# ToniChopp/ECAMP

Hardware: AMD Instinct MI355X
Metric: pretrain image-report pairs/sec (ViT-B/16, 224^2, seq=128) (higher is better)
Workload: dtype bf16

## Files before the change

### ecamp_amd/csrc/attention.h

```cpp
#pragma once
#include "common.h"

struct AttnArgs {
    const void* q; const void* k; const void* v; void* o;
    const void* dout; void* dq; void* dk; void* dv;
    float* lse; float* delta;
    const int32_t* key_mask;
    long q_sb, q_st, q_sh, k_sb, k_st, k_sh, v_sb, v_st, v_sh, o_sb, o_st, o_sh;
    long dq_sb, dq_st, dq_sh, dk_sb, dk_st, dk_sh, dv_sb, dv_st, dv_sh, do_sb, do_st, do_sh;
    int B, H, Tq, Tk;
    float scale, drop_p;
    uint64_t seed, offset;
    unsigned char* drop_bits;
};

#define NEG_BIG (-1.0e30f)

#define LDS_MAX (160 * 1024)

static inline int attn_kch(int Tk) { return Tk <= 64 ? 1 : Tk <= 128 ? 2 : Tk <= 256 ? 4 : 0; }

static inline size_t head_lds_bytes(int Tq, int Tk, int hd, bool backward, bool bits) {
    const int nkp = ((Tk + 15) / 16 + 1) / 2, nqp = ((Tq + 15) / 16 + 1) / 2;
    const size_t prow = (size_t)(backward && nqp > nkp ? nqp : nkp) * 32;
    return 2 * prow * (2 * hd) + (backward ? 3 : 1) * prow * sizeof(float) + (backward && bits ? 32 * prow : 0);
}

enum AttnFamily { ATTN_HEAD, ATTN_RESIDENT_FWD, ATTN_STREAM, ATTN_LONG, ATTN_F32 };
typedef void (*AttnKernel)(AttnArgs);
struct AttnLaunch {
    AttnFamily family;
    int n, block;
    struct Kernel { AttnKernel fn; dim3 grid; size_t lds, optin; } k[2];
};
#define ATTN_HD_SWITCH(hd, F, ...) ((hd) == 32 ? F<32>(__VA_ARGS__) : (hd) == 64 ? F<64>(__VA_ARGS__) : F<128>(__VA_ARGS__))

ECAMP_HIDDEN AttnLaunch attn16_select(int B, int H, int Tq, int Tk, int hd, bool mask_or_dropout, bool bits, bool backward);
ECAMP_HIDDEN void attn_launch(const AttnLaunch& l, const AttnArgs& a, hipStream_t st);
void attn_set_head_mode(int on);
```

### ecamp_amd/csrc/attention_bf16.hip

```cpp
#include "attention.h"
#include <type_traits>

#ifdef ATTN_TS
__device__ long long attn_ts_buf[8 * 8192];
#define ATTN_STAMP(i) do { if (threadIdx.x == 0 && blockIdx.x < 8192) attn_ts_buf[blockIdx.x * 8 + (i)] = wall_clock64(); } while (0)
#else
#define ATTN_STAMP(i) do { } while (0)
#endif

typedef __attribute__((ext_vector_type(4))) short v4s16;
typedef hw_h16x8 bf16x8_t;

#define MFMA(a, b, c) ECAMP_MFMA_16x16x32(a, b, c)

#define ATTN_LOG2E 1.4426950408889634f
#define ATTN_LN2 0.6931471805599453f
__device__ __forceinline__ float attn_exp2(float x) { return __builtin_amdgcn_exp2f(x); }

template <int HD> struct TileCfg { static constexpr int PB = HD * 2 + 32; static constexpr int BYTES = 64 * PB; };

template <int HD>
__device__ __forceinline__ void stage_tile(unsigned char* lds, const bf16_t* base, long st, int r0, int nrows, int tid) {
    constexpr int CPR = HD / 8, PB = TileCfg<HD>::PB;
#pragma unroll
// ... 269 lines not shown
            const int4 km = *reinterpret_cast<const int4*>(KM + jt * 16 + 4 * g);
            const int kmv[4] = {km.x, km.y, km.z, km.w};
            float ds[4], dm[4] = {1.f, 1.f, 1.f, 1.f};
            if (a.drop_p > 0.f) attn_drop4(a, (uint64_t)bh * a.Tq + qi, c * 64 + jt * 16 + 4 * g, inv_keep, dm);
#pragma unroll
            for (int r = 0; r < 4; ++r) {
                const bool ok = qok && kmv[r] != 0;
                float p = ok ? attn_exp2(fmaf(s[r], sc2, -lse2)) : 0.f;
                ds[r] = p * (dp[r] * dm[r] - dl);
            }
            ptile_write4(st, li, jt * 16 + 4 * g, ds);
        }
        __builtin_amdgcn_s_waitcnt(0xc07f);
        __builtin_amdgcn_wave_barrier();
#pragma unroll
        for (int kk = 0; kk < 2; ++kk) {
            bf16x8 sf = ptile_frag(st, li, kk * 4 + g);
#pragma unroll
            for (int dt = 0; dt < HD / 16; ++dt) dq[dt] = MFMA(frag_tr<HD>(KT, dt * 16, kk * 32, lane), sf, dq[dt]);
        }
    }
    if (qok) {
#pragma unroll
        for (int dt = 0; dt < HD / 16; ++dt) store4(dqb + (long)qi * a.dq_st + dt * 16 + 4 * g, dq[dt], a.scale);
    }
}

template <int HD, int KCH>
__global__ __launch_bounds__(256) void attn16_bwd_dq_kernel(AttnArgs a) {
    const int nact = min(4, (a.Tq - (int)blockIdx.x * 64 + 15) >> 4);
    if (nact < 4) {
        if ((int)(threadIdx.x >> 6) >= nact) return;
        attn16_bwd_dq_body<HD, KCH, true>(a, nact * 64);
    } else {
        attn16_bwd_dq_body<HD, KCH, false>(a, 256);
    }
}

template <int HD, bool PART>
__device__ __forceinline__ void attn16_bwd_dkv_body(const AttnArgs& a, int nthr) {
    extern __shared__ __attribute__((aligned(16))) unsigned char smem[];
    unsigned char* QT = smem;
    unsigned char* GT = smem + TileCfg<HD>::BYTES;
    unsigned char* PT = smem + 2 * TileCfg<HD>::BYTES;
    unsigned char* ST = PT + 4 * 2048;
    float* LS = reinterpret_cast<float*>(ST + 4 * 2048);
    const int tid = threadIdx.x, lane = tid & 63, wave = tid >> 6, li = lane & 15, g = lane >> 4;
    const int b = blockIdx.y / a.H, h = blockIdx.y % a.H;
    const int j0 = blockIdx.x * 64 + wave * 16;
    const long bh = (long)b * a.H + h;
    const bf16_t* qb = reinterpret_cast<const bf16_t*>(a.q) + b * a.q_sb + h * a.q_sh;
    const bf16_t* kb = reinterpret_cast<const bf16_t*>(a.k) + b * a.k_sb + h * a.k_sh;
    const bf16_t* vb = reinterpret_cast<const bf16_t*>(a.v) + b * a.v_sb + h * a.v_sh;
    const bf16_t* gb = reinterpret_cast<const bf16_t*>(a.dout) + b * a.do_sb + h * a.do_sh;
    bf16_t* dkb = reinterpret_cast<bf16_t*>(a.dk) + b * a.dk_sb + h * a.dk_sh;
    bf16_t* dvb = reinterpret_cast<bf16_t*>(a.dv) + b * a.dv_sb + h * a.dv_sh;

    bf16x8 kf[HD / 32], vf[HD / 32];
    load_row_frags<HD>(kf, kb, a.k_st, j0, a.Tk, lane);
    load_row_frags<HD>(vf, vb, a.v_st, j0, a.Tk, lane);
    const int kj = j0 + li;
    const bool jok = kj < a.Tk && (a.key_mask == nullptr || a.key_mask[(long)b * a.Tk + kj] != 0);
    const float inv_keep = a.drop_p > 0.f ? 1.0f / (1.0f - a.drop_p) : 1.0f, sc2 = a.scale * ATTN_LOG2E;
    f32x4 dk[HD / 16], dv[HD / 16];
#pragma unroll
    for (int dt = 0; dt < HD / 16; ++dt) dk[dt] = dv[dt] = (f32x4){0.f, 0.f, 0.f, 0.f};
    unsigned char* pt = PT + wave * 2048;
    unsigned char* st = ST + wave * 2048;
    const int nqc = (a.Tq + 63) / 64;
#pragma unroll 1
    for (int c = 0; c < nqc; ++c) {
        __syncthreads();
        if (PART) {
            stage_tile_n<HD>(QT, qb, a.q_st, c * 64, a.Tq, tid, nthr);
            stage_tile_n<HD>(GT, gb, a.do_st, c * 64, a.Tq, tid, nthr);
        } else {
            stage_tile<HD>(QT, qb, a.q_st, c * 64, a.Tq, tid);
            stage_tile<HD>(GT, gb, a.do_st, c * 64, a.Tq, tid);
        }
        if (tid < 64) {
            const int i = c * 64 + tid;
            LS[tid] = i < a.Tq ? a.lse[bh * a.Tq + i] * ATTN_LOG2E : 0.f;
            LS[64 + tid] = i < a.Tq ? a.delta[bh * a.Tq + i] : 0.f;
        }
        __syncthreads();
#pragma unroll
        for (int it = 0; it < 4; ++it) {
            f32x4 s = {0.f, 0.f, 0.f, 0.f}, dp = {0.f, 0.f, 0.f, 0.f};
#pragma unroll
            for (int ks = 0; ks < HD / 32; ++ks) {
                s = MFMA(frag_rows<HD>(QT, it * 16 + li, ks * 4 + g), kf[ks], s);
                dp = MFMA(frag_rows<HD>(GT, it * 16 + li, ks * 4 + g), vf[ks], dp);
            }
            float pd[4], ds[4], dm[4] = {1.f, 1.f, 1.f, 1.f};
            if (a.drop_p > 0.f) attn_drop4_col(a, (uint64_t)bh * a.Tq + (c * 64 + it * 16 + 4 * g), kj, li, inv_keep, dm);
            const f32x4 lse4 = *reinterpret_cast<const f32x4*>(LS + it * 16 + 4 * g);
            const f32x4 dl4 = *reinterpret_cast<const f32x4*>(LS + 64 + it * 16 + 4 * g);
#pragma unroll
            for (int r = 0; r < 4; ++r) {
                int i = c * 64 + it * 16 + 4 * g + r;
                bool ok = jok && i < a.Tq;
                float p = ok ? attn_exp2(fmaf(s[r], sc2, -lse4[r])) : 0.f;
                pd[r] = p * dm[r];
                ds[r] = p * (dp[r] * dm[r] - dl4[r]);
            }
            ptile_write4(pt, li, it * 16 + 4 * g, pd);
            ptile_write4(st, li, it * 16 + 4 * g, ds);
        }
        __builtin_amdgcn_s_waitcnt(0xc07f);
        __builtin_amdgcn_wave_barrier();
#pragma unroll
        for (int kk = 0; kk < 2; ++kk) {
            bf16x8 pf = ptile_frag(pt, li, kk * 4 + g), sf = ptile_frag(st, li, kk * 4 + g);
#pragma unroll
            for (int dt = 0; dt < HD / 16; ++dt) {
                dv[dt] = MFMA(frag_tr<HD>(GT, dt * 16, kk * 32, lane), pf, dv[dt]);
                dk[dt] = MFMA(frag_tr<HD>(QT, dt * 16, kk * 32, lane), sf, dk[dt]);
            }
        }
    }
    if (kj < a.Tk) {
#pragma unroll
        for (int dt = 0; dt < HD / 16; ++dt) {
            store4(dkb + (long)kj * a.dk_st + dt * 16 + 4 * g, dk[dt], a.scale);
            store4(dvb + (long)kj * a.dv_st + dt * 16 + 4 * g, dv[dt], 1.0f);
        }
    }
}

template <int HD>
__global__ __launch_bounds__(256) void attn16_bwd_dkv_kernel(AttnArgs a) {
    const int nact = min(4, (a.Tk - (int)blockIdx.x * 64 + 15) >> 4);
    if (nact < 4) {
        if ((int)(threadIdx.x >> 6) >= nact) return;
        attn16_bwd_dkv_body<HD, true>(a, nact * 64);
    } else {
        attn16_bwd_dkv_body<HD, false>(a, 256);
    }
}

template <int HD, int KCH>
__global__ __launch_bounds__(256) void attn16r_fwd_kernel(AttnArgs a) {
    extern __shared__ __attribute__((aligned(16))) unsigned char smem[];
    constexpr int TB = TileCfg<HD>::BYTES;
    unsigned char* KT = smem;
    unsigned char* VT = smem + KCH * TB;
    unsigned char* PT = smem + 2 * KCH * TB;
    const int tid = threadIdx.x, lane = tid & 63, wave = tid >> 6, li = lane & 15, g = lane >> 4;
    const int b = blockIdx.x / a.H, h = blockIdx.x % a.H;
    const long bh = blockIdx.x;
    const bf16_t* qb = reinterpret_cast<const bf16_t*>(a.q) + b * a.q_sb + h * a.q_sh;
    const bf16_t* kb = reinterpret_cast<const bf16_t*>(a.k) + b * a.k_sb + h * a.k_sh;
    const bf16_t* vb = reinterpret_cast<const bf16_t*>(a.v) + b * a.v_sb + h * a.v_sh;
    bf16_t* ob = reinterpret_cast<bf16_t*>(a.o) + b * a.o_sb + h * a.o_sh;
#pragma unroll
    for (int c = 0; c < KCH; ++c) {
        stage_tile<HD>(KT + c * TB, kb, a.k_st, c * 64, a.Tk, tid);
        stage_tile<HD>(VT + c * TB, vb, a.v_st, c * 64, a.Tk, tid);
    }
    __syncthreads();
    const float inv_keep = a.drop_p > 0.f ? 1.0f / (1.0f - a.drop_p) : 1.0f;
    unsigned char* pt = PT + wave * 2048;
    unsigned long long kok = 0ull;
#pragma unroll
    for (int t = 0; t < KCH * 4; ++t)
#pragma unroll
        for (int r = 0; r < 4; ++r) {
            int j = t * 16 + 4 * g + r;
            bool ok = j < a.Tk && (a.key_mask == nullptr || a.key_mask[(long)b * a.Tk + j] != 0);
            kok |= (unsigned long long)(ok ? 1 : 0) << (t * 4 + r);
        }
    for (int q0 = wave * 16; q0 < a.Tq; q0 += 64) {
        bf16x8 qf[HD / 32];
        load_row_frags<HD>(qf, qb, a.q_st, q0, a.Tq, lane);
        f32x4 s[KCH * 4];
#pragma unroll
        for (int c = 0; c < KCH; ++c)
#pragma unroll
            for (int jt = 0; jt < 4; ++jt) {
                f32x4 acc = {0.f, 0.f, 0.f, 0.f};
#pragma unroll
                for (int ks = 0; ks < HD / 32; ++ks) acc = MFMA(frag_rows<HD>(KT + c * TB, jt * 16 + li, ks * 4 + g), qf[ks], acc);
                s[c * 4 + jt] = acc;
            }
        float mx = NEG_BIG;
#pragma unroll
        for (int t = 0; t < KCH * 4; ++t)
#pragma unroll
            for (int r = 0; r < 4; ++r) {
                s[t][r] = ((kok >> (t * 4 + r)) & 1ull) ? s[t][r] * (a.scale * ATTN_LOG2E) : NEG_BIG;
                mx = fmaxf(mx, s[t][r]);
            }
        mx = red4_max(mx);
        const float mxs = fmaxf(mx, -1e29f);
        float sum = 0.f;
#pragma unroll
        for (int t = 0; t < KCH * 4; ++t)
#pragma unroll
            for (int r = 0; r < 4; ++r) {
                float p = attn_exp2(s[t][r] - mxs);
                s[t][r] = p;
                sum += p;
            }
        sum = red4_sum(sum);
        const int qi = q0 + li;
        if (g == 0 && qi < a.Tq) a.lse[bh * a.Tq + qi] = (mx + __log2f(sum)) * ATTN_LN2;
        const float inv = 1.0f / sum;
        f32x4 o[HD / 16];
#pragma unroll
        for (int dt = 0; dt < HD / 16; ++dt) o[dt] = (f32x4){0.f, 0.f, 0.f, 0.f};
#pragma unroll
        for (int c = 0; c < KCH; ++c) {
#pragma unroll
            for (int jt = 0; jt < 4; ++jt) {
                float p[4];
#pragma unroll
                for (int r = 0; r < 4; ++r) p[r] = s[c * 4 + jt][r] * inv;
                if (a.drop_p > 0.f) {
                    float dm[4];
                    attn_drop4(a, (uint64_t)bh * a.Tq + qi, c * 64 + jt * 16 + 4 * g, inv_keep, dm);
#pragma unroll
                    for (int r = 0; r < 4; ++r) p[r] *= dm[r];
                }
                ptile_write4(pt, li, jt * 16 + 4 * g, p);
            }
            __builtin_amdgcn_s_waitcnt(0xc07f);
            __builtin_amdgcn_wave_barrier();
#pragma unroll
            for (int kk = 0; kk < 2; ++kk) {
                bf16x8 pf = ptile_frag(pt, li, kk * 4 + g);
#pragma unroll
                for (int dt = 0; dt < HD / 16; ++dt) o[dt] = MFMA(frag_tr<HD>(VT + c * TB, dt * 16, kk * 32, lane), pf, o[dt]);
            }
            __builtin_amdgcn_s_waitcnt(0xc07f);
            __builtin_amdgcn_wave_barrier();
        }
        if (qi < a.Tq) {
#pragma unroll
            for (int dt = 0; dt < HD / 16; ++dt) store4(ob + (long)qi * a.o_st + dt * 16 + 4 * g, o[dt], 1.0f);
        }
    }
}

template <int HD> struct HeadCfg {
    static constexpr int RB = HD * 2, CPR = HD / 8;
    static constexpr unsigned long long KEYS = HD == 32 ? 0x3033030132330101ull : HD == 64 ? 0x6056142366024421ull : 0xE0CA8436CE0A3864ull;
};
template <int HD> __device__ __forceinline__ int hswz(int row) { return (int)((HeadCfg<HD>::KEYS >> (4 * (row & 15))) & 15ull); }
template <int HD> __device__ __forceinline__ unsigned haddr(int row, int chunk) {
    return (unsigned)(row * HeadCfg<HD>::RB + ((chunk ^ hswz<HD>(row)) << 4));
}
template <int HD>
__device__ __forceinline__ void head_stage(unsigned char* img, const bf16_t* base, long st, int nrows, int prow, int tid, int nthr) {
    constexpr int CPR = HeadCfg<HD>::CPR;
    const int n = prow * CPR;
    for (int i0 = tid; i0 < n; i0 += 4 * nthr) {
        uint4 v[4];
#pragma unroll
        for (int u = 0; u < 4; ++u) {
            const int idx = i0 + u * nthr, row = idx / CPR, ch = idx % CPR;
            v[u] = (idx < n && row < nrows) ? *reinterpret_cast<const uint4*>(base + (long)row * st + ch * 8) : make_uint4(0, 0, 0, 0);
        }
#pragma unroll
        for (int u = 0; u < 4; ++u) {
            const int idx = i0 + u * nthr, row = idx / CPR, ch = idx % CPR;
            if (idx < n) *reinterpret_cast<uint4*>(img + haddr<HD>(row, ch)) = v[u];
        }
    }
}
template <int HD, int U>
__device__ __forceinline__ void head_stage_pair(unsigned char* imgA, const bf16_t* baseA, long stA, unsigned char* imgB, const bf16_t* baseB, long stB,
                                                int nrows, int prow, int tid, int nthr) {
    constexpr int CPR = HeadCfg<HD>::CPR;
    const int n = prow * CPR;
    for (int i0 = tid; i0 < n; i0 += U * nthr) {
        uint4 va[U], vb[U];
#pragma unroll
        for (int u = 0; u < U; ++u) {
            const int idx = i0 + u * nthr, row = idx / CPR, ch = idx % CPR;
            const bool in = idx < n && row < nrows;
            va[u] = in ? *reinterpret_cast<const uint4*>(baseA + (long)row * stA + ch * 8) : make_uint4(0, 0, 0, 0);
            vb[u] = in ? *reinterpret_cast<const uint4*>(baseB + (long)row * stB + ch * 8) : make_uint4(0, 0, 0, 0);
        }
#pragma unroll
        for (int u = 0; u < U; ++u) {
            const int idx = i0 + u * nthr, row = idx / CPR, ch = idx % CPR;
            if (idx < n) {
                *reinterpret_cast<uint4*>(imgA + haddr<HD>(row, ch)) = va[u];
                *reinterpret_cast<uint4*>(imgB + haddr<HD>(row, ch)) = vb[u];
            }
        }
    }
}
typedef float f32x2 __attribute__((ext_vector_type(2)));
__device__ __forceinline__ f32x2 hexp2(f32x2 x) { return (f32x2){attn_exp2(x[0]), attn_exp2(x[1])}; }
__device__ __forceinline__ uint32_t hpk(f32x2 v) { return pack_bf16x2(v[0], v[1]); }
__device__ __forceinline__ bf16x8 hpack8(const float (&v)[8]) {
    const uint4 u = make_uint4(pack_bf16x2(v[0], v[1]), pack_bf16x2(v[2], v[3]), pack_bf16x2(v[4], v[5]), pack_bf16x2(v[6], v[7]));
    return __builtin_bit_cast(bf16x8, u);
}
__device__ __forceinline__ void head_key_bias(float* KB, const AttnArgs& a, int b, int prow, int tid, int nthr) {
    for (int j = tid; j < prow; j += nthr)
        KB[j] = (j < a.Tk && (a.key_mask == nullptr || a.key_mask[(long)b * a.Tk + j] != 0)) ? 0.f : NEG_BIG;
}
template <int HD> struct HeadOff {
    unsigned fr[HD / 32];
    unsigned tr[HD / 16];
    __device__ __forceinline__ HeadOff(int li, int g) {
#pragma unroll
        for (int ks = 0; ks < HD / 32; ++ks) fr[ks] = haddr<HD>(li, ks * 4 + g);
#pragma unroll
        for (int dt = 0; dt < HD / 16; ++dt) {
            const int cb = (dt * 16 + (li & 3) * 4) * 2;
            tr[dt] = haddr<HD>(4 * g + (li >> 2), cb >> 4) + (cb & 15);
        }
    }
};
template <int HD> __device__ __forceinline__ bf16x8 hfr(const unsigned char* img, const HeadOff<HD>& o, int t, int ks) {
    return *reinterpret_cast<const bf16x8*>(img + o.fr[ks] + t * (16 * HeadCfg<HD>::RB));
}
template <int HD> __device__ __forceinline__ bf16x8 htr(const unsigned char* img, const HeadOff<HD>& o, int pp, int dt) {
    const unsigned char* p = img + o.tr[dt] + pp * (32 * HeadCfg<HD>::RB);
    v4s16 lo = __builtin_amdgcn_ds_read_tr16_b64_v4i16((v4s16 __attribute__((address_space(3)))*)(p));
    v4s16 hi = __builtin_amdgcn_ds_read_tr16_b64_v4i16((v4s16 __attribute__((address_space(3)))*)(p + 16 * HeadCfg<HD>::RB));
    return (bf16x8){lo[0], lo[1], lo[2], lo[3], hi[0], hi[1], hi[2], hi[3]};
}

template <int HD, int FLAGS>
__global__ __launch_bounds__(512, 4) void attn_head_fwd_kernel(AttnArgs a) {
    extern __shared__ __attribute__((aligned(16))) unsigned char smem[];
    constexpr int RB = HeadCfg<HD>::RB;
    const int nthr = blockDim.x, nw = nthr >> 6;
    const int nkp = (((a.Tk + 15) >> 4) + 1) >> 1, prow = nkp * 32;
    const int pfull = FLAGS ? 0 : a.Tk >> 5;
    unsigned char* KI = smem;
    unsigned char* VI = smem + prow * RB;
    float* KB = reinterpret_cast<float*>(smem + 2 * prow * RB);
    const int tid = threadIdx.x, lane = tid & 63, wave = tid >> 6, li = lane & 15, g = lane >> 4;
    const int b = blockIdx.x / a.H, h = blockIdx.x % a.H;
    const long bh = blockIdx.x;
    const bf16_t* qb = reinterpret_cast<const bf16_t*>(a.q) + b * a.q_sb + h * a.q_sh;
    const bf16_t* kb = reinterpret_cast<const bf16_t*>(a.k) + b * a.k_sb + h * a.k_sh;
    const bf16_t* vb = reinterpret_cast<const bf16_t*>(a.v) + b * a.v_sb + h * a.v_sh;
    bf16_t* ob = reinterpret_cast<bf16_t*>(a.o) + b * a.o_sb + h * a.o_sh;
    bf16x8 qf[HD / 32];
    if (wave * 16 < a.Tq) load_row_frags<HD>(qf, qb, a.q_st, wave * 16, a.Tq, lane);
    head_stage_pair<HD, 4>(KI, kb, a.k_st, VI, vb, a.v_st, a.Tk, prow, tid, nthr);
    head_key_bias(KB, a, b, prow, tid, nthr);
    __syncthreads();
    const HeadOff<HD> off(li, g);
    const float sc2 = a.scale * ATTN_LOG2E;
    const float inv_keep = a.drop_p > 0.f ? 1.0f / (1.0f - a.drop_p) : 1.0f;
    for (int q0 = wave * 16; q0 < a.Tq; q0 += nw * 16) {
        auto scores = [&](int t, bool biased) {
            f32x4 acc = {0.f, 0.f, 0.f, 0.f};
#pragma unroll
            for (int ks = 0; ks < HD / 32; ++ks) acc = MFMA(hfr<HD>(KI, off, t, ks), qf[ks], acc);
            if (biased) {
                const f32x4 kb4 = *reinterpret_cast<const f32x4*>(KB + t * 16 + 4 * g);
#pragma unroll
                for (int r = 0; r < 4; ++r) acc[r] = fmaf(acc[r], sc2, kb4[r]);
            } else {
#pragma unroll
                for (int r = 0; r < 4; ++r) acc[r] *= sc2;
            }
            return acc;
        };
        float mx = NEG_BIG;
#pragma unroll 2
        for (int pp = 0; pp < pfull; ++pp) {
            const f32x4 s0 = scores(2 * pp, false), s1 = scores(2 * pp + 1, false);
            mx = fmaxf(fmaxf(fmaxf(mx, fmaxf(s0[0], s0[1])), fmaxf(s0[2], s0[3])), fmaxf(fmaxf(s1[0], s1[1]), fmaxf(s1[2], s1[3])));
        }
#pragma unroll 1
        for (int pp = pfull; pp < nkp; ++pp) {
            const f32x4 s0 = scores(2 * pp, true), s1 = scores(2 * pp + 1, true);
            mx = fmaxf(fmaxf(fmaxf(mx, fmaxf(s0[0], s0[1])), fmaxf(s0[2], s0[3])), fmaxf(fmaxf(s1[0], s1[1]), fmaxf(s1[2], s1[3])));
        }
        mx = red4_max(mx);
        const float mxs = fmaxf(mx, -1e29f);
        const int qi = q0 + li;
        float sum = 0.f;
        f32x4 o[HD / 16];
#pragma unroll
        for (int dt = 0; dt < HD / 16; ++dt) o[dt] = (f32x4){0.f, 0.f, 0.f, 0.f};
        auto pair = [&](int pp, bool biased) {
            const f32x4 s0 = scores(2 * pp, biased), s1 = scores(2 * pp + 1, biased);
            float p[8];
#pragma unroll
            for (int r = 0; r < 4; ++r) {
                p[r] = attn_exp2(s0[r] - mxs);
                p[4 + r] = attn_exp2(s1[r] - mxs);
                sum += p[r] + p[4 + r];
            }
            if (FLAGS && a.drop_p > 0.f) {
                float dm[4], dn[4];
                if ((a.Tk & 7) == 0) {
                    const bool odd = (g & 1) != 0;
                    const uint64_t e8 = ((((uint64_t)bh * a.Tq + qi) * (uint64_t)a.Tk) >> 3) + (uint64_t)(pp * 4 + (odd ? 2 : 0) + (g >> 1));
                    const uint4 P = philox4x32(a.seed, a.offset, e8);
                    const uint32_t r0 = (uint32_t)__builtin_amdgcn_ds_swizzle((int)(odd ? P.x : P.z), 0x401f);
                    const uint32_t r1 = (uint32_t)__builtin_amdgcn_ds_swizzle((int)(odd ? P.y : P.w), 0x401f);
                    const uint32_t wa0 = odd ? r0 : P.x, wa1 = odd ? r1 : P.y, wb0 = odd ? P.z : r0, wb1 = odd ? P.w : r1;
                    const uint32_t thr = dropout_thr(a.drop_p);
                    dm[0] = dropout_pick(wa0, 0, thr, inv_keep); dm[1] = dropout_pick(wa0, 1, thr, inv_keep);
                    dm[2] = dropout_pick(wa1, 0, thr, inv_keep); dm[3] = dropout_pick(wa1, 1, thr, inv_keep);
                    dn[0] = dropout_pick(wb0, 0, thr, inv_keep); dn[1] = dropout_pick(wb0, 1, thr, inv_keep);
                    dn[2] = dropout_pick(wb1, 0, thr, inv_keep); dn[3] = dropout_pick(wb1, 1, thr, inv_keep);
                } else {
                    attn_drop4(a, (uint64_t)bh * a.Tq + qi, pp * 32 + 4 * g, inv_keep, dm);
                    attn_drop4(a, (uint64_t)bh * a.Tq + qi, pp * 32 + 16 + 4 * g, inv_keep, dn);
                }
                unsigned bits = 0;
#pragma unroll
                for (int r = 0; r < 4; ++r) {
                    p[r] *= dm[r];
                    p[4 + r] *= dn[r];
                    bits |= (dm[r] != 0.f ? 1u << r : 0u) | (dn[r] != 0.f ? 16u << r : 0u);
                }
                if (a.drop_bits && qi < a.Tq) a.drop_bits[(((long)bh * a.Tq + qi) * 4 + g) * 8 + pp] = (unsigned char)bits;
            }
            const bf16x8 pf = hpack8(p);
#pragma unroll
            for (int dt = 0; dt < HD / 16; ++dt) o[dt] = MFMA(htr<HD>(VI, off, pp, dt), pf, o[dt]);
        };
#pragma unroll 2
        for (int pp = 0; pp < pfull; ++pp) pair(pp, false);
#pragma unroll 1
        for (int pp = pfull; pp < nkp; ++pp) pair(pp, true);
        sum = red4_sum(sum);
        if (qi < a.Tq) {
            if (g == 0) a.lse[bh * a.Tq + qi] = (mxs + __log2f(sum)) * ATTN_LN2;
            const float inv = sum > 0.f ? 1.0f / sum : 0.f;
#pragma unroll
            for (int dt = 0; dt < HD / 16; ++dt) store4(ob + (long)qi * a.o_st + dt * 16 + 4 * g, o[dt], inv);
        }
        if (q0 + nw * 16 < a.Tq) load_row_frags<HD>(qf, qb, a.q_st, q0 + nw * 16, a.Tq, lane);
    }
}

template <int HD, int FLAGS>
__global__ __launch_bounds__(256, (FLAGS == 0 && HD == 32) ? 5 : (FLAGS == 0 && HD == 64) ? 4 : 2) void attn_head_bwd_kernel(AttnArgs a) {
    extern __shared__ __attribute__((aligned(16))) unsigned char smem[];
    constexpr int RB = HeadCfg<HD>::RB;
    const int nthr = blockDim.x, nw = nthr >> 6;
    const int nkp = (((a.Tk + 15) >> 4) + 1) >> 1, nqp = (((a.Tq + 15) >> 4) + 1) >> 1, prow = max(nkp, nqp) * 32;
    const int pfull = FLAGS ? 0 : a.Tk >> 5;
    unsigned char* XI = smem;
    unsigned char* YI = smem + prow * RB;
    float* KB = reinterpret_cast<float*>(smem + 2 * prow * RB);
    float* LS = KB + prow;
    float* DL = LS + prow;
    unsigned char* MB = reinterpret_cast<unsigned char*>(DL + prow);
    const int tid = threadIdx.x, lane = tid & 63, wave = tid >> 6, li = lane & 15, g = lane >> 4;
    const int b = blockIdx.x / a.H, h = blockIdx.x % a.H;
    const long bh = blockIdx.x;
    const bool use_bits = FLAGS && a.drop_p > 0.f && a.drop_bits != nullptr;
    const bf16_t* qb = reinterpret_cast<const bf16_t*>(a.q) + b * a.q_sb + h * a.q_sh;
    const bf16_t* kb = reinterpret_cast<const bf16_t*>(a.k) + b * a.k_sb + h * a.k_sh;
    const bf16_t* vb = reinterpret_cast<const bf16_t*>(a.v) + b * a.v_sb + h * a.v_sh;
    const bf16_t* ob = reinterpret_cast<const bf16_t*>(a.o) + b * a.o_sb + h * a.o_sh;
    const bf16_t* gb = reinterpret_cast<const bf16_t*>(a.dout) + b * a.do_sb + h * a.do_sh;
    bf16_t* dqb = reinterpret_cast<bf16_t*>(a.dq) + b * a.dq_sb + h * a.dq_sh;
    bf16_t* dkb = reinterpret_cast<bf16_t*>(a.dk) + b * a.dk_sb + h * a.dk_sh;
    bf16_t* dvb = reinterpret_cast<bf16_t*>(a.dv) + b * a.dv_sb + h * a.dv_sh;
    const float sc2 = a.scale * ATTN_LOG2E;
    const float inv_keep = a.drop_p > 0.f ? 1.0f / (1.0f - a.drop_p) : 1.0f;
    const HeadOff<HD> off(li, g);

    ATTN_STAMP(0);
    bf16x8 qf[HD / 32], gf[HD / 32], of[HD / 32];
    float lse_c = 0.f;
    uint2 mw = make_uint2(0u, 0u);
    auto load_q = [&](int q0, bf16x8 (&q_)[HD / 32], bf16x8 (&g_)[HD / 32], bf16x8 (&o_)[HD / 32], float& l_) {
        load_row_frags<HD>(q_, qb, a.q_st, q0, a.Tq, lane);
        load_row_frags<HD>(g_, gb, a.do_st, q0, a.Tq, lane);
        load_row_frags<HD>(o_, ob, a.o_st, q0, a.Tq, lane);
        l_ = q0 + li < a.Tq ? a.lse[bh * a.Tq + q0 + li] : 0.f;
        if (use_bits && q0 + li < a.Tq) mw = *reinterpret_cast<const uint2*>(a.drop_bits + (((long)bh * a.Tq + q0 + li) * 4 + g) * 8);
    };
    if (wave * 16 < a.Tq) load_q(wave * 16, qf, gf, of, lse_c);
    head_stage_pair<HD, (HD == 128 ? 8 : 4)>(XI, kb, a.k_st, YI, vb, a.v_st, a.Tk, prow, tid, nthr);
    head_key_bias(KB, a, b, prow, tid, nthr);
    for (int i = ((a.Tq + 15) & ~15) + tid; i < prow; i += nthr) { LS[i] = 1e30f; DL[i] = 0.f; }
    __syncthreads();
    ATTN_STAMP(1);
    for (int q0 = wave * 16; q0 < a.Tq; q0 += nw * 16) {
        float dl = 0.f;
#pragma unroll
        for (int ks = 0; ks < HD / 32; ++ks)
#pragma unroll
            for (int e = 0; e < 8; ++e) dl += bf2f((bf16_t)gf[ks][e]) * bf2f((bf16_t)of[ks][e]);
        dl = red4_sum(dl);
        const int qi = q0 + li;
        const bool qok = qi < a.Tq;
        const float lse2 = qok ? lse_c * ATTN_LOG2E : 1e30f;
        if (g == 0) {
            LS[qi] = lse2;
            DL[qi] = qok ? dl : 0.f;
            if (qok && a.delta) a.delta[bh * a.Tq + qi] = dl;
        }
        f32x4 dq[HD / 16];
#pragma unroll
        for (int dt = 0; dt < HD / 16; ++dt) dq[dt] = (f32x4){0.f, 0.f, 0.f, 0.f};
        auto soft = [&](int pp, int hf, bool biased, const f32x4& s, const f32x4& dp, uint32_t& w0, uint32_t& w1) __attribute__((always_inline)) {
            const int t = 2 * pp + hf;
            f32x2 e0 = {s[0], s[1]}, e1 = {s[2], s[3]}, d0 = {dp[0], dp[1]}, d1 = {dp[2], dp[3]};
            const f32x2 sc = {sc2, sc2}, nl = {-lse2, -lse2}, dlv = {dl, dl};
            if (biased) {
                const f32x4 kb4 = *reinterpret_cast<const f32x4*>(KB + t * 16 + 4 * g);
                e0 = e0 * sc + ((f32x2){kb4[0], kb4[1]} + nl);
                e1 = e1 * sc + ((f32x2){kb4[2], kb4[3]} + nl);
            } else {
                e0 = e0 * sc + nl;
                e1 = e1 * sc + nl;
            }
            if (FLAGS && a.drop_p > 0.f) {
                float dm[4];
                if (use_bits) {
                    const unsigned nib = ((pp < 4 ? mw.x : mw.y) >> (8 * (pp & 3) + 4 * hf)) & 15u;
#pragma unroll
                    for (int r = 0; r < 4; ++r) dm[r] = (nib >> r) & 1u ? inv_keep : 0.f;
                } else {
                    attn_drop4(a, (uint64_t)bh * a.Tq + qi, t * 16 + 4 * g, inv_keep, dm);
                }
                d0 *= (f32x2){dm[0], dm[1]};
                d1 *= (f32x2){dm[2], dm[3]};
            }
            w0 = hpk(hexp2(e0) * (d0 - dlv));
            w1 = hpk(hexp2(e1) * (d1 - dlv));
        };
        auto pair = [&](int pp, bool biased) {
            uint32_t dsp[4];
            {
#pragma unroll
                for (int hf = 0; hf < 2; ++hf) {
                    const int t = 2 * pp + hf;
                    f32x4 s = {0.f, 0.f, 0.f, 0.f}, dp = {0.f, 0.f, 0.f, 0.f};
#pragma unroll
                    for (int ks = 0; ks < HD / 32; ++ks) {
                        s = MFMA(hfr<HD>(XI, off, t, ks), qf[ks], s);
                        dp = MFMA(hfr<HD>(YI, off, t, ks), gf[ks], dp);
                    }
                    soft(pp, hf, biased, s, dp, dsp[2 * hf], dsp[2 * hf + 1]);
                }
                const bf16x8 sf = __builtin_bit_cast(bf16x8, make_uint4(dsp[0], dsp[1], dsp[2], dsp[3]));
#pragma unroll
                for (int dt = 0; dt < HD / 16; ++dt) dq[dt] = MFMA(htr<HD>(XI, off, pp, dt), sf, dq[dt]);
            }
        };
#pragma unroll 2
        for (int pp = 0; pp < pfull; ++pp) pair(pp, false);
#pragma unroll 1
        for (int pp = pfull; pp < nkp; ++pp) pair(pp, true);
        if (qok) {
#pragma unroll
            for (int dt = 0; dt < HD / 16; ++dt) store4(dqb + (long)qi * a.dq_st + dt * 16 + 4 * g, dq[dt], a.scale);
        }
        if (q0 + nw * 16 < a.Tq) load_q(q0 + nw * 16, qf, gf, of, lse_c);
    }
    ATTN_STAMP(2);
    bf16x8 kf[HD / 32], vf[HD / 32];
    if (wave * 16 < a.Tk) {
        load_row_frags<HD>(kf, kb, a.k_st, wave * 16, a.Tk, lane);
        load_row_frags<HD>(vf, vb, a.v_st, wave * 16, a.Tk, lane);
    }
    __syncthreads();
    ATTN_STAMP(3);
    head_stage_pair<HD, (HD == 128 ? 8 : 4)>(XI, qb, a.q_st, YI, gb, a.do_st, a.Tq, prow, tid, nthr);
    if (use_bits) {
        for (int i = tid; i < a.Tq * 4; i += nthr) {
            const int row = i >> 2, gg = i & 3;
            const uint2 w = *reinterpret_cast<const uint2*>(a.drop_bits + ((long)bh * a.Tq * 4 + i) * 8);
#pragma unroll
            for (int pp = 0; pp < 8; ++pp) MB[(gg * 8 + pp) * prow + row] = (unsigned char)(((pp < 4 ? w.x : w.y) >> (8 * (pp & 3))) & 255u);
        }
    }
    __syncthreads();
    ATTN_STAMP(4);
    for (int j0 = wave * 16; j0 < a.Tk; j0 += nw * 16) {
        const int kj = j0 + li;
        const bool jok = KB[kj] == 0.f;
        const f32x2 kb2 = {KB[kj], KB[kj]};
        const unsigned char* mcol = MB + ((((kj & 15) >> 2) * 8 + (kj >> 5)) * prow);
        const int mbit = 4 * ((kj >> 4) & 1) + (kj & 3);
        f32x4 dk[HD / 16], dv[HD / 16];
#pragma unroll
        for (int dt = 0; dt < HD / 16; ++dt) dk[dt] = dv[dt] = (f32x4){0.f, 0.f, 0.f, 0.f};
#pragma unroll 2
        for (int ip = 0; ip < nqp; ++ip) {
            uint32_t pdp[4], dsp[4];
            auto soft2 = [&](int hf, const f32x4& s, const f32x4& dp) __attribute__((always_inline)) {
                const int it = 2 * ip + hf;
                const f32x4 lse4 = *reinterpret_cast<const f32x4*>(LS + it * 16 + 4 * g);
                const f32x4 dl4 = *reinterpret_cast<const f32x4*>(DL + it * 16 + 4 * g);
                const f32x2 sc = {sc2, sc2};
                f32x2 d0 = {dp[0], dp[1]}, d1 = {dp[2], dp[3]};
                f32x2 e0 = (f32x2){s[0], s[1]} * sc - (f32x2){lse4[0], lse4[1]}, e1 = (f32x2){s[2], s[3]} * sc - (f32x2){lse4[2], lse4[3]};
                if (FLAGS) { e0 += kb2; e1 += kb2; }
                f32x2 p0 = hexp2(e0);
                f32x2 p1 = hexp2(e1);
                if (FLAGS && a.drop_p > 0.f) {
                    float dm[4];
                    if (use_bits) {
                        const unsigned m4 = *reinterpret_cast<const unsigned*>(mcol + it * 16 + 4 * g) >> mbit;
#pragma unroll
                        for (int r = 0; r < 4; ++r) dm[r] = (m4 >> (8 * r)) & 1u ? inv_keep : 0.f;
                    } else {
                        attn_drop4_col(a, (uint64_t)bh * a.Tq + (it * 16 + 4 * g), kj, li, inv_keep, dm);
                    }
                    const f32x2 m0 = {dm[0], dm[1]}, m1 = {dm[2], dm[3]};
                    d0 *= m0; d1 *= m1;
                    pdp[2 * hf] = hpk(p0 * m0);
                    pdp[2 * hf + 1] = hpk(p1 * m1);
                } else {
                    pdp[2 * hf] = hpk(p0);
                    pdp[2 * hf + 1] = hpk(p1);
                }
                dsp[2 * hf] = hpk(p0 * (d0 - (f32x2){dl4[0], dl4[1]}));
                dsp[2 * hf + 1] = hpk(p1 * (d1 - (f32x2){dl4[2], dl4[3]}));
            };
            {
#pragma unroll
                for (int hf = 0; hf < 2; ++hf) {
                    const int it = 2 * ip + hf;
                    f32x4 s = {0.f, 0.f, 0.f, 0.f}, dp = {0.f, 0.f, 0.f, 0.f};
#pragma unroll
                    for (int ks = 0; ks < HD / 32; ++ks) {
                        s = MFMA(hfr<HD>(XI, off, it, ks), kf[ks], s);
                        dp = MFMA(hfr<HD>(YI, off, it, ks), vf[ks], dp);
                    }
                    soft2(hf, s, dp);
                }
                const bf16x8 pf = __builtin_bit_cast(bf16x8, make_uint4(pdp[0], pdp[1], pdp[2], pdp[3]));
                const bf16x8 sf = __builtin_bit_cast(bf16x8, make_uint4(dsp[0], dsp[1], dsp[2], dsp[3]));
#pragma unroll
                for (int dt = 0; dt < HD / 16; ++dt) {
                    dv[dt] = MFMA(htr<HD>(YI, off, ip, dt), pf, dv[dt]);
                    dk[dt] = MFMA(htr<HD>(XI, off, ip, dt), sf, dk[dt]);
                }
            }
        }
        if (kj < a.Tk) {
            const float mk = jok ? a.scale : 0.f, mv = jok ? 1.0f : 0.f;
#pragma unroll
            for (int dt = 0; dt < HD / 16; ++dt) {
                store4(dkb + (long)kj * a.dk_st + dt * 16 + 4 * g, dk[dt], mk);
                store4(dvb + (long)kj * a.dv_st + dt * 16 + 4 * g, dv[dt], mv);
            }
        }
        if (j0 + nw * 16 < a.Tk) {
            load_row_frags<HD>(kf, kb, a.k_st, j0 + nw * 16, a.Tk, lane);
            load_row_frags<HD>(vf, vb, a.v_st, j0 + nw * 16, a.Tk, lane);
        }
    }
    ATTN_STAMP(5);
}

static long g_head_launches = 0;
extern "C" int64_t ecamp_attn_head_launches(void) { return g_head_launches; }
void attn_set_head_mode(int on) { ecamp_opt_set("attn_head", on); }
static int head_waves(int tiles, int cap) {
    const int env = ecamp_opt(OPT_ATTN_WAVES);
    if (env > 0) cap = env;
    return tiles < cap ? tiles : cap;
}
template <int HD>
static AttnLaunch select16(int B, int H, int Tq, int Tk, bool flags, bool bits, bool backward) {
    static_assert(HeadCfg<HD>::RB == 2 * HD, "head_lds_bytes (attention.h) states the row size of the head images");
    AttnLaunch l = {};
    l.n = 1;
    l.block = 256;
    const int nqt = (Tq + 15) / 16, nkt = (Tk + 15) / 16;
    const size_t head = head_lds_bytes(Tq, Tk, HD, backward, bits);
    if (ecamp_opt(OPT_ATTN_HEAD) != 0 && head <= LDS_MAX) {
        l.family = ATTN_HEAD;
        l.block = 64 * (backward ? head_waves(nkt > nqt ? nkt : nqt, 4) : head_waves(nqt, 8));
        const AttnKernel fn = backward ? (flags ? attn_head_bwd_kernel<HD, 1> : attn_head_bwd_kernel<HD, 0>)
                                       : (flags ? attn_head_fwd_kernel<HD, 1> : attn_head_fwd_kernel<HD, 0>);
        l.k[0] = {fn, dim3(B * H), head, LDS_MAX};
        return l;
    }
    const dim3 qgrid(ceil_div(Tq, 64), B * H), kgrid(ceil_div(Tk, 64), B * H);
    const size_t stream = (size_t)2 * TileCfg<HD>::BYTES + 4 * 2048 + 64 * sizeof(int);
    const int kch = attn_kch(Tk);
    if (backward) {
        l.family = ATTN_STREAM;
        l.n = 2;
        const AttnKernel dq = kch == 1 ? attn16_bwd_dq_kernel<HD, 1> : kch == 2 ? attn16_bwd_dq_kernel<HD, 2> : kch == 4 ? attn16_bwd_dq_kernel<HD, 4>
                                                                                                                       : attn16_bwd_dq_kernel<HD, 0>;
        l.k[0] = {dq, qgrid, stream, 0};
        l.k[1] = {attn16_bwd_dkv_kernel<HD>, kgrid, (size_t)2 * TileCfg<HD>::BYTES + 8 * 2048 + 128 * sizeof(float), 0};
        return l;
    }
    if (Tk > 128) {
        l.family = ATTN_LONG;
        l.k[0] = {attn16_fwd_long_kernel<HD>, qgrid, stream, 0};
        return l;
    }
    l.family = ATTN_RESIDENT_FWD;
    const size_t shm = (size_t)2 * kch * TileCfg<HD>::BYTES + 4 * 2048;
    l.k[0] = {kch == 1 ? attn16r_fwd_kernel<HD, 1> : attn16r_fwd_kernel<HD, 2>, dim3(B * H), shm, shm};
    return l;
}
AttnLaunch attn16_select(int B, int H, int Tq, int Tk, int hd, bool mask_or_dropout, bool bits, bool backward) {
    return ATTN_HD_SWITCH(hd, select16, B, H, Tq, Tk, mask_or_dropout, bits, backward);
}

void attn_launch(const AttnLaunch& l, const AttnArgs& a, hipStream_t st) {
    static const void* seen[64];
    static int n_seen = 0;
    for (int i = 0; i < l.n; ++i) {
        const AttnLaunch::Kernel& k = l.k[i];
        const void* fn = reinterpret_cast<const void*>(k.fn);
        bool known = k.optin <= 48 * 1024;
        for (int s = 0; s < n_seen && !known; ++s) known = seen[s] == fn;
        if (!known) {
            (void)hipFuncSetAttribute(fn, hipFuncAttributeMaxDynamicSharedMemorySize, (int)k.optin);
            if (n_seen < 64) seen[n_seen++] = fn;
        }
        hipLaunchKernelGGL(k.fn, k.grid, dim3(l.block), k.lds, st, a);
    }
    if (l.family == ATTN_HEAD) ++g_head_launches;
}
```

### ecamp_amd/csrc/core.hip

```cpp
#include "common.h"
#include "attention.h"
#include "options.h"
#include "../../include/ecamp_hip.h"
#include <atomic>
#include <stdarg.h>
#include <stdlib.h>

thread_local char g_ecamp_err[512] = {0};

int ecamp_set_error(int code, const char* fmt, ...) {
    va_list ap;
    va_start(ap, fmt);
    vsnprintf(g_ecamp_err, sizeof(g_ecamp_err), fmt, ap);
    va_end(ap);
    return code;
}

extern "C" const char* ecamp_last_error(void) { return g_ecamp_err; }
extern "C" int ecamp_abi_version(void) { return ECAMP_ABI_VERSION; }
extern "C" int ecamp_half_format(void) { return ECAMP_HALF_IS_F16; }

#define OPT_UNREAD (INT_MIN + 1)
struct OptRow {
    const char* name; const char* env; int def; int (*set)(int);
    std::atomic<int> value{OPT_ENV};
    std::atomic<int> env_value{OPT_UNREAD};
};
static OptRow g_opts[OPT_COUNT] = {
              {"q8_mode", "ECAMP_GEMM_Q8", -1, [](int v) { return v == 0 || v == 2 ? v : -1; }},
               {"q8_sch", "ECAMP_Q8_SCH", 7, [](int v) { return v >= 0 ? v : OPT_ENV; }},
             {"q16_mode", "ECAMP_Q16", 1, [](int v) { return v >= 0 && v <= 3 ? v : OPT_ENV; }},
                {nullptr, "ECAMP_F8_Q8", 1, nullptr},
         {nullptr, "ECAMP_Q8_MIN_ITEMS", OPT_AUTO, nullptr},
          {"q8_bwd_grid", "ECAMP_Q8_BWD_GRID", 0, [](int v) { return v > 0 ? v : OPT_ENV; }},
             {"p8_wgrad", nullptr, 1, [](int v) { return v ? 1 : 0; }},
     {"p8_wgrad_reserve_cus", nullptr, 0, [](int v) { return v < 0 ? 0 : v; }},
          {nullptr, "ECAMP_WGRAD_ITEMS", 0, nullptr},
           {nullptr, "ECAMP_WGRAD_PLAN", 1, nullptr},
      {nullptr, "ECAMP_WGRAD_GROUP_CUS", 0, nullptr},
        {nullptr, "ECAMP_GEMM_GRID_CAP", 0, nullptr},
            {"attn_head", "ECAMP_ATTN_HEAD", 1, [](int v) { return v < 0 ? OPT_ENV : v ? 1 : 0; }},
           {nullptr, "ECAMP_ATTN_WAVES", 0, nullptr},
               {nullptr, "ECAMP_LN_BWD", 0, nullptr},
            {nullptr, "ECAMP_CE_KERNEL", 1, nullptr},
            {nullptr, "ECAMP_SR_BLOCKS", 512, nullptr},
};
int ecamp_opt_default(EcampOpt id) { return g_opts[id].def; }
int ecamp_opt(EcampOpt id) {
    OptRow& o = g_opts[id];
    const int s = o.value.load(std::memory_order_relaxed);
    if (s != OPT_ENV) return s;
    int e = o.env_value.load(std::memory_order_relaxed);
    if (e == OPT_UNREAD) {
        const char* txt = o.env ? getenv(o.env) : nullptr;
        e = txt ? atoi(txt) : o.def;
        o.env_value.store(e, std::memory_order_relaxed);
    }
    return e;
}
bool ecamp_opt_set(const char* name, int value) {
    for (OptRow& o : g_opts)
        if (o.name && strcmp(name, o.name) == 0) {
            o.value.store(o.set(value), std::memory_order_relaxed);
            return true;
        }
    return false;
}
extern "C" int ecamp_set_option(const char* name, int32_t value) {
    ECAMP_CHECK_ARG(name != nullptr, "set_option: null name");
    if (strcmp(name, "attn_head") == 0) { attn_set_head_mode(value); return 0; }
    if (ecamp_opt_set(name, value)) return 0;
    return ecamp_set_error(-1, "set_option: unknown option '%s'", name);
}

__global__ void dev_spin_kernel(long long cycles) {
    const long long t0 = clock64();
    while (clock64() - t0 < cycles) {}
}
extern "C" int ecamp_dev_spin(int32_t blocks, int32_t threads, int64_t cycles, hipStream_t stream) {
    ECAMP_CHECK_ARG(blocks > 0 && threads > 0 && threads <= 1024 && cycles >= 0, "dev_spin: bad arguments");
    hipLaunchKernelGGL(dev_spin_kernel, dim3(blocks), dim3(threads), 0, stream, (long long)cycles);
    ECAMP_LAUNCH_CHECK();
    return 0;
}
```

### ecamp_amd/csrc/options.h

```cpp
#pragma once
#include <limits.h>

enum EcampOpt {
    OPT_Q8_MODE, OPT_Q8_SCH, OPT_Q16_MODE, OPT_F8_Q8, OPT_Q8_MIN_ITEMS, OPT_Q8_BWD_GRID, OPT_P8_WGRAD, OPT_P8_WGRAD_RESERVE,
    OPT_WGRAD_ITEMS, OPT_WGRAD_PLAN, OPT_WGRAD_GROUP_CUS, OPT_GEMM_GRID_CAP, OPT_ATTN_HEAD, OPT_ATTN_WAVES, OPT_LN_BWD, OPT_CE_KERNEL,
    OPT_SR_BLOCKS, OPT_COUNT
};
#define OPT_ENV INT_MIN
#define OPT_AUTO INT_MIN

#define ECAMP_HIDDEN __attribute__((visibility("hidden")))
ECAMP_HIDDEN int ecamp_opt(EcampOpt id);
ECAMP_HIDDEN int ecamp_opt_default(EcampOpt id);
ECAMP_HIDDEN bool ecamp_opt_set(const char* name, int value);
```

Before: 7344.

## Skip fully masked key tiles in head attention forward and backward

Builds a per-block bitmask of 16-key tiles that contain at least one unmasked key, computed from the key-bias array with wave ballots. The forward and backward head kernels skip score, softmax, and dK/dV work for dead tiles. Skipped tiles get zero gradients written directly, and dropout bits are still generated so the saved mask stays consistent. This targets padded text sequences (seq=128) where trailing key tiles are all padding. It adds ballot overhead and branch divergence between waves, and it depends on padding being grouped into whole tiles.

```diff
diff --git a/ecamp_amd/csrc/attention.h b/ecamp_amd/csrc/attention.h
--- a/ecamp_amd/csrc/attention.h
+++ b/ecamp_amd/csrc/attention.h
@@ -12,6 +12,7 @@
     float scale, drop_p;
     uint64_t seed, offset;
     unsigned char* drop_bits;
+    int key_bounds;
 };
 
 #define NEG_BIG (-1.0e30f)
@@ -26,11 +27,14 @@
     return 2 * prow * (2 * hd) + (backward ? 3 : 1) * prow * sizeof(float) + (backward && bits ? 32 * prow : 0);
 }
 
+static inline bool attn_key_bounds_on(int Tk, bool flags, int opt) { return flags && opt != 0 && (Tk + 15) / 16 <= 64; }
+
 enum AttnFamily { ATTN_HEAD, ATTN_RESIDENT_FWD, ATTN_STREAM, ATTN_LONG, ATTN_F32 };
 typedef void (*AttnKernel)(AttnArgs);
 struct AttnLaunch {
     AttnFamily family;
     int n, block;
+    int key_bounds;
     struct Kernel { AttnKernel fn; dim3 grid; size_t lds, optin; } k[2];
 };
 #define ATTN_HD_SWITCH(hd, F, ...) ((hd) == 32 ? F<32>(__VA_ARGS__) : (hd) == 64 ? F<64>(__VA_ARGS__) : F<128>(__VA_ARGS__))
diff --git a/ecamp_amd/csrc/attention_bf16.hip b/ecamp_amd/csrc/attention_bf16.hip
--- a/ecamp_amd/csrc/attention_bf16.hip
+++ b/ecamp_amd/csrc/attention_bf16.hip
@@ -595,6 +595,25 @@
 __device__ __forceinline__ void head_key_bias(float* KB, const AttnArgs& a, int b, int prow, int tid, int nthr) {
     for (int j = tid; j < prow; j += nthr)
         KB[j] = (j < a.Tk && (a.key_mask == nullptr || a.key_mask[(long)b * a.Tk + j] != 0)) ? 0.f : NEG_BIG;
+}
+__device__ __forceinline__ unsigned long long head_live_tiles(const float* KB, int ntile, int lane, int on) {
+    if (!on) return ~0ull;
+    unsigned lo = 0u, hi = 0u;
+    const int n = ntile * 16;
+    for (int c = 0; c * 8 < ntile; ++c) {
+        const int j0 = c * 128 + lane, j1 = j0 + 64;
+        const float b0 = KB[min(j0, n - 1)], b1 = KB[min(j1, n - 1)];
+        const unsigned long long m0 = __ballot(j0 < n && b0 == 0.f), m1 = __ballot(j1 < n && b1 == 0.f);
+        unsigned byte = 0u;
+#pragma unroll
+        for (int t = 0; t < 4; ++t)
+            byte |= (((m0 >> (16 * t)) & 0xffffull) != 0ull ? 1u << t : 0u) | (((m1 >> (16 * t)) & 0xffffull) != 0ull ? 16u << t : 0u);
+        if (c < 4) lo |= byte << (8 * c); else hi |= byte << (8 * (c - 4));
+    }
+    lo = (unsigned)__builtin_amdgcn_readfirstlane((int)lo);
+    hi = (unsigned)__builtin_amdgcn_readfirstlane((int)hi);
+    const unsigned long long live = ((unsigned long long)hi << 32) | lo;
+    return live != 0ull ? live : ~0ull;
 }
 template <int HD> struct HeadOff {
     unsigned fr[HD / 32];
@@ -644,6 +663,8 @@
     const HeadOff<HD> off(li, g);
     const float sc2 = a.scale * ATTN_LOG2E;
     const float inv_keep = a.drop_p > 0.f ? 1.0f / (1.0f - a.drop_p) : 1.0f;
+    const unsigned long long live = FLAGS ? head_live_tiles(KB, 2 * nkp, lane, a.key_bounds) : ~0ull;
+    auto pair_live = [&](int pp) { return ((live >> ((2 * pp) & 63)) & 3ull) != 0ull; };
     for (int q0 = wave * 16; q0 < a.Tq; q0 += nw * 16) {
         auto scores = [&](int t, bool biased) {
             f32x4 acc = {0.f, 0.f, 0.f, 0.f};
@@ -667,6 +688,7 @@
         }
 #pragma unroll 1
         for (int pp = pfull; pp < nkp; ++pp) {
+            if (FLAGS && !pair_live(pp)) continue;
             const f32x4 s0 = scores(2 * pp, true), s1 = scores(2 * pp + 1, true);
             mx = fmaxf(fmaxf(fmaxf(mx, fmaxf(s0[0], s0[1])), fmaxf(s0[2], s0[3])), fmaxf(fmaxf(s1[0], s1[1]), fmaxf(s1[2], s1[3])));
         }
@@ -677,6 +699,28 @@
         f32x4 o[HD / 16];
 #pragma unroll
         for (int dt = 0; dt < HD / 16; ++dt) o[dt] = (f32x4){0.f, 0.f, 0.f, 0.f};
+        auto keep8 = [&](int pp, float (&dm)[4], float (&dn)[4]) {
+            if ((a.Tk & 7) == 0) {
+                const bool odd = (g & 1) != 0;
+                const uint64_t e8 = ((((uint64_t)bh * a.Tq + qi) * (uint64_t)a.Tk) >> 3) + (uint64_t)(pp * 4 + (odd ? 2 : 0) + (g >> 1));
+                const uint4 P = philox4x32(a.seed, a.offset, e8);
+                const uint32_t r0 = (uint32_t)__builtin_amdgcn_ds_swizzle((int)(odd ? P.x : P.z), 0x401f);
+                const uint32_t r1 = (uint32_t)__builtin_amdgcn_ds_swizzle((int)(odd ? P.y : P.w), 0x401f);
+                const uint32_t wa0 = odd ? r0 : P.x, wa1 = odd ? r1 : P.y, wb0 = odd ? P.z : r0, wb1 = odd ? P.w : r1;
+                const uint32_t thr = dropout_thr(a.drop_p);
+                dm[0] = dropout_pick(wa0, 0, thr, inv_keep); dm[1] = dropout_pick(wa0, 1, thr, inv_keep);
+                dm[2] = dropout_pick(wa1, 0, thr, inv_keep); dm[3] = dropout_pick(wa1, 1, thr, inv_keep);
+                dn[0] = dropout_pick(wb0, 0, thr, inv_keep); dn[1] = dropout_pick(wb0, 1, thr, inv_keep);
+                dn[2] = dropout_pick(wb1, 0, thr, inv_keep); dn[3] = dropout_pick(wb1, 1, thr, inv_keep);
+            } else {
+                attn_drop4(a, (uint64_t)bh * a.Tq + qi, pp * 32 + 4 * g, inv_keep, dm);
+                attn_drop4(a, (uint64_t)bh * a.Tq + qi, pp * 32 + 16 + 4 * g, inv_keep, dn);
+            }
+            unsigned bits = 0;
+#pragma unroll
+            for (int r = 0; r < 4; ++r) bits |= (dm[r] != 0.f ? 1u << r : 0u) | (dn[r] != 0.f ? 16u << r : 0u);
+            if (a.drop_bits && qi < a.Tq) a.drop_bits[(((long)bh * a.Tq + qi) * 4 + g) * 8 + pp] = (unsigned char)bits;
+        };
         auto pair = [&](int pp, bool biased) {
             const f32x4 s0 = scores(2 * pp, biased), s1 = scores(2 * pp + 1, biased);
             float p[8];
@@ -688,30 +732,12 @@
             }
             if (FLAGS && a.drop_p > 0.f) {
                 float dm[4], dn[4];
-                if ((a.Tk & 7) == 0) {
-                    const bool odd = (g & 1) != 0;
-                    const uint64_t e8 = ((((uint64_t)bh * a.Tq + qi) * (uint64_t)a.Tk) >> 3) + (uint64_t)(pp * 4 + (odd ? 2 : 0) + (g >> 1));
-                    const uint4 P = philox4x32(a.seed, a.offset, e8);
-                    const uint32_t r0 = (uint32_t)__builtin_amdgcn_ds_swizzle((int)(odd ? P.x : P.z), 0x401f);
-                    const uint32_t r1 = (uint32_t)__builtin_amdgcn_ds_swizzle((int)(odd ? P.y : P.w), 0x401f);
-                    const uint32_t wa0 = odd ? r0 : P.x, wa1 = odd ? r1 : P.y, wb0 = odd ? P.z : r0, wb1 = odd ? P.w : r1;
-                    const uint32_t thr = dropout_thr(a.drop_p);
-                    dm[0] = dropout_pick(wa0, 0, thr, inv_keep); dm[1] = dropout_pick(wa0, 1, thr, inv_keep);
-                    dm[2] = dropout_pick(wa1, 0, thr, inv_keep); dm[3] = dropout_pick(wa1, 1, thr, inv_keep);
-                    dn[0] = dropout_pick(wb0, 0, thr, inv_keep); dn[1] = dropout_pick(wb0, 1, thr, inv_keep);
-                    dn[2] = dropout_pick(wb1, 0, thr, inv_keep); dn[3] = dropout_pick(wb1, 1, thr, inv_keep);
-                } else {
-                    attn_drop4(a, (uint64_t)bh * a.Tq + qi, pp * 32 + 4 * g, inv_keep, dm);
-                    attn_drop4(a, (uint64_t)bh * a.Tq + qi, pp * 32 + 16 + 4 * g, inv_keep, dn);
-                }
-                unsigned bits = 0;
+                keep8(pp, dm, dn);
 #pragma unroll
                 for (int r = 0; r < 4; ++r) {
                     p[r] *= dm[r];
                     p[4 + r] *= dn[r];
-                    bits |= (dm[r] != 0.f ? 1u << r : 0u) | (dn[r] != 0.f ? 16u << r : 0u);
                 }
-                if (a.drop_bits && qi < a.Tq) a.drop_bits[(((long)bh * a.Tq + qi) * 4 + g) * 8 + pp] = (unsigned char)bits;
             }
             const bf16x8 pf = hpack8(p);
 #pragma unroll
@@ -720,7 +746,16 @@
 #pragma unroll 2
         for (int pp = 0; pp < pfull; ++pp) pair(pp, false);
 #pragma unroll 1
-        for (int pp = pfull; pp < nkp; ++pp) pair(pp, true);
+        for (int pp = pfull; pp < nkp; ++pp) {
+            if (FLAGS && !pair_live(pp)) {
+                if (a.drop_p > 0.f && a.drop_bits) {
+                    float dm[4], dn[4];
+                    keep8(pp, dm, dn);
+                }
+                continue;
+            }
+            pair(pp, true);
+        }
         sum = red4_sum(sum);
         if (qi < a.Tq) {
             if (g == 0) a.lse[bh * a.Tq + qi] = (mxs + __log2f(sum)) * ATTN_LN2;
@@ -778,6 +813,9 @@
     for (int i = ((a.Tq + 15) & ~15) + tid; i < prow; i += nthr) { LS[i] = 1e30f; DL[i] = 0.f; }
     __syncthreads();
     ATTN_STAMP(1);
+    const unsigned long long live = FLAGS ? head_live_tiles(KB, 2 * nkp, lane, a.key_bounds) : ~0ull;
+    auto pair_live = [&](int pp) { return ((live >> ((2 * pp) & 63)) & 3ull) != 0ull; };
+    auto tile_live = [&](int j0) { return !FLAGS || ((live >> ((j0 >> 4) & 63)) & 1ull) != 0ull; };
     for (int q0 = wave * 16; q0 < a.Tq; q0 += nw * 16) {
         float dl = 0.f;
 #pragma unroll
@@ -845,7 +883,10 @@
 #pragma unroll 2
         for (int pp = 0; pp < pfull; ++pp) pair(pp, false);
 #pragma unroll 1
-        for (int pp = pfull; pp < nkp; ++pp) pair(pp, true);
+        for (int pp = pfull; pp < nkp; ++pp) {
+            if (FLAGS && !pair_live(pp)) continue;
+            pair(pp, true);
+        }
         if (qok) {
 #pragma unroll
             for (int dt = 0; dt < HD / 16; ++dt) store4(dqb + (long)qi * a.dq_st + dt * 16 + 4 * g, dq[dt], a.scale);
@@ -854,10 +895,13 @@
     }
     ATTN_STAMP(2);
     bf16x8 kf[HD / 32], vf[HD / 32];
-    if (wave * 16 < a.Tk) {
-        load_row_frags<HD>(kf, kb, a.k_st, wave * 16, a.Tk, lane);
-        load_row_frags<HD>(vf, vb, a.v_st, wave * 16, a.Tk, lane);
-    }
+    auto load_kv = [&](int j0) {
+        if (j0 < a.Tk && tile_live(j0)) {
+            load_row_frags<HD>(kf, kb, a.k_st, j0, a.Tk, lane);
+            load_row_frags<HD>(vf, vb, a.v_st, j0, a.Tk, lane);
+        }
+    };
+    load_kv(wave * 16);
     __syncthreads();
     ATTN_STAMP(3);
     head_stage_pair<HD, (HD == 128 ? 8 : 4)>(XI, qb, a.q_st, YI, gb, a.do_st, a.Tq, prow, tid, nthr);
@@ -873,6 +917,17 @@
     ATTN_STAMP(4);
     for (int j0 = wave * 16; j0 < a.Tk; j0 += nw * 16) {
         const int kj = j0 + li;
+        if (!tile_live(j0)) {
+            if (kj < a.Tk) {
+#pragma unroll
+                for (int dt = 0; dt < HD / 16; ++dt) {
+                    *reinterpret_cast<uint2*>(dkb + (long)kj * a.dk_st + dt * 16 + 4 * g) = make_uint2(0u, 0u);
+                    *reinterpret_cast<uint2*>(dvb + (long)kj * a.dv_st + dt * 16 + 4 * g) = make_uint2(0u, 0u);
+                }
+            }
+            load_kv(j0 + nw * 16);
+            continue;
+        }
         const bool jok = KB[kj] == 0.f;
         const f32x2 kb2 = {KB[kj], KB[kj]};
         const unsigned char* mcol = MB + ((((kj & 15) >> 2) * 8 + (kj >> 5)) * prow);
@@ -942,10 +997,7 @@
                 store4(dvb + (long)kj * a.dv_st + dt * 16 + 4 * g, dv[dt], mv);
             }
         }
-        if (j0 + nw * 16 < a.Tk) {
-            load_row_frags<HD>(kf, kb, a.k_st, j0 + nw * 16, a.Tk, lane);
-            load_row_frags<HD>(vf, vb, a.v_st, j0 + nw * 16, a.Tk, lane);
-        }
+        load_kv(j0 + nw * 16);
     }
     ATTN_STAMP(5);
 }
@@ -972,6 +1024,7 @@
         const AttnKernel fn = backward ? (flags ? attn_head_bwd_kernel<HD, 1> : attn_head_bwd_kernel<HD, 0>)
                                        : (flags ? attn_head_fwd_kernel<HD, 1> : attn_head_fwd_kernel<HD, 0>);
         l.k[0] = {fn, dim3(B * H), head, LDS_MAX};
+        l.key_bounds = attn_key_bounds_on(Tk, flags, ecamp_opt(OPT_ATTN_KEY_BOUNDS));
         return l;
     }
     const dim3 qgrid(ceil_div(Tq, 64), B * H), kgrid(ceil_div(Tk, 64), B * H);
@@ -1000,9 +1053,11 @@
     return ATTN_HD_SWITCH(hd, select16, B, H, Tq, Tk, mask_or_dropout, bits, backward);
 }
 
-void attn_launch(const AttnLaunch& l, const AttnArgs& a, hipStream_t st) {
+void attn_launch(const AttnLaunch& l, const AttnArgs& args, hipStream_t st) {
     static const void* seen[64];
     static int n_seen = 0;
+    AttnArgs a = args;
+    a.key_bounds = l.key_bounds;
     for (int i = 0; i < l.n; ++i) {
         const AttnLaunch::Kernel& k = l.k[i];
         const void* fn = reinterpret_cast<const void*>(k.fn);
diff --git a/ecamp_amd/csrc/core.hip b/ecamp_amd/csrc/core.hip
--- a/ecamp_amd/csrc/core.hip
+++ b/ecamp_amd/csrc/core.hip
@@ -41,7 +41,8 @@
         {nullptr, "ECAMP_GEMM_GRID_CAP", 0, nullptr},
             {"attn_head", "ECAMP_ATTN_HEAD", 1, [](int v) { return v < 0 ? OPT_ENV : v ? 1 : 0; }},
            {nullptr, "ECAMP_ATTN_WAVES", 0, nullptr},
-               {nullptr, "ECAMP_LN_BWD", 0, nullptr},
+      {"attn_key_bounds", "ECAMP_ATTN_KEY_BOUNDS", 1, [](int v) { return v < 0 ? OPT_ENV : v ? 1 : 0; }},
+              {nullptr, "ECAMP_LN_BWD", 0, nullptr},
             {nullptr, "ECAMP_CE_KERNEL", 1, nullptr},
             {nullptr, "ECAMP_SR_BLOCKS", 512, nullptr},
 };
diff --git a/ecamp_amd/csrc/options.h b/ecamp_amd/csrc/options.h
--- a/ecamp_amd/csrc/options.h
+++ b/ecamp_amd/csrc/options.h
@@ -3,8 +3,8 @@
 
 enum EcampOpt {
     OPT_Q8_MODE, OPT_Q8_SCH, OPT_Q16_MODE, OPT_F8_Q8, OPT_Q8_MIN_ITEMS, OPT_Q8_BWD_GRID, OPT_P8_WGRAD, OPT_P8_WGRAD_RESERVE,
-    OPT_WGRAD_ITEMS, OPT_WGRAD_PLAN, OPT_WGRAD_GROUP_CUS, OPT_GEMM_GRID_CAP, OPT_ATTN_HEAD, OPT_ATTN_WAVES, OPT_LN_BWD, OPT_CE_KERNEL,
-    OPT_SR_BLOCKS, OPT_COUNT
+    OPT_WGRAD_ITEMS, OPT_WGRAD_PLAN, OPT_WGRAD_GROUP_CUS, OPT_GEMM_GRID_CAP, OPT_ATTN_HEAD, OPT_ATTN_WAVES, OPT_ATTN_KEY_BOUNDS, OPT_LN_BWD,
+    OPT_CE_KERNEL, OPT_SR_BLOCKS, OPT_COUNT
 };
 #define OPT_ENV INT_MIN
 #define OPT_AUTO INT_MIN
```

Result: slower. 6311 (-14.1%).
